# connortannahill/MM-ADMM

Measured on AMD Instinct MI355X. Metric: ADMM iterations/sec on 1M-node 2D mesh; achieved HBM GB/s in SpMV, higher is better.
Workload: dtype f64

## Files before the change

### mm-admm_amd/csrc/host/engine.cpp

```cpp
#include <algorithm>
#include <chrono>
#include <cmath>
#include <cstring>
#include <limits>
#include <memory>
#include <mutex>
#include <string>
#include <vector>

#include "../../../include/mmx_sparse.h"
#include "../kernels/admm_kernels.h"
#include "../kernels/regrid_kernels.h"
#include "comm.h"
#include "common.h"
#include "partition.h"

#define MMX_SP(expr)                                                                     \
  do {                                                                                   \
    const int rc_ = (expr);                                                              \
    if (rc_ != MMADMM_OK) throw ::mmx::Error(rc_, std::string(#expr) + ": " + mmadmm_last_error()); \
  } while (0)

namespace mmx {

// ... 264 lines not shown
  void step(int nIters, double tol, double* Ih, int* itersOut) override {
    if (nIters < 1) throw Error(MMADMM_ERR_INVALID, "step: nIters must be >= 1");
    if (regridEachStep_) regrid(stepsTaken_ * prm_.dt);
    ensureResults(nIters);
    const bool timing = timing_;
    hipEvent_t eStep0 = nullptr, eStep1 = nullptr;
    if (timing) {
      eStep0 = nextEvent();
      MMX_HIP(hipEventRecord(eStep0, st_));
    }
    const double dtOverTau = prm_.dt / prm_.tau;
    const bool fusePred = zFromX_ && fusePred_ && !wave2d_ && !(prm_.grad_use || stepsTaken_ <= 2);
    if (prm_.grad_use || stepsTaken_ <= 2) {
      int nb = 0;
      launch_grad_simplex<D>(m_, x_.p, gs_.p, true, partA_.p, &nb, st_);
      exchange(1);
      launch_predict<D>(m_, 0, gs_.p, x_.p, xPrev_.p, xBar_.p, dtOverTau, st_);
    } else if (!fusePred) {
      launch_predict<D>(m_, 1, nullptr, x_.p, xPrev_.p, xBar_.p, dtOverTau, st_);
    }
    const double* zsrc = stepsTaken_ == 0 ? xPrev_.p : xBar_.p;
    const bool zFromX = zFromX_ && !wave2d_;
    if (!stepTaken_) clearU();
    if (zFromX)
      m_.zx = zsrc;
    else
      launch_gather_z<D>(m_, zsrc, z_.p, st_);
    gcacheValid_ = false;
    if (!zFromX) m_.zx = nullptr;
    StepScalars sc{prm_.tau, prm_.dt * prm_.dt, w_, dtOverTau};
    int nbx = 0, nbp = 0;
    if (fusePred) {
      m_.predPrev = xPrev_.p;
      m_.predBar = xBar_.p;
    }
    PackZX pz;
    if (zFromX) {
      pz.F = F_.p;
      pz.zx = zsrc;
      if (fusePred) {
        pz.x = x_.p;
        pz.xPrev = xPrev_.p;
      }
    }
    xupdateHalo(sc, &nbx, false, false, pz);
    m_.predPrev = m_.predBar = nullptr;
    const bool early = tol >= 0;
    int done = 0;
    double primal = 0, dual = 0;
    const bool deferRed = !early && nIters <= kDeferMax;
    const size_t slice = maxBlocks_ * kNumPartials;
    if (deferRed && partA_.n < slice * nIters) partA_.alloc(slice * std::max(nIters, 10));
    int firstDeferred = 0;
    for (int i = 0; i < nIters; ++i) {
      hipEvent_t a0 = nullptr, a1 = nullptr, b1 = nullptr;
      if (timing) {
        a0 = nextEvent();
        MMX_HIP(hipEventRecord(a0, st_));
      }
      const bool firstProx = !hessComputed_;
      const bool swapB = prox_double_buffered(D, wave2d_) && hessComputed_;
      if (hessComputed_) {
        tiePar_ ^= 1;
        std::swap(m_.tieCount, m_.tieStale);
      }
      launch_prox<D>(m_, !hessComputed_, gcacheValid_, early ? tol / 100 : 1e-3 / 100, x_.p, z_.p, uPtr(), B_.p,
                     swapB ? B2_.p : B_.p, partA_.p + (deferRed ? slice * i : 0), &nbp, st_);
      m_.zx = nullptr;
      if (swapB) std::swap(B_.p, B2_.p);
      gcacheValid_ = true;
      if (timing) {
        a1 = nextEvent();
        MMX_HIP(hipEventRecord(a1, st_));
      }
      hessComputed_ = true;
      stepTaken_ = true;
      const bool resid = early || i == nIters - 1;
      xupdateHalo(sc, &nbx, resid, true, PackZX{});
      if (timing) {
        b1 = nextEvent();
        MMX_HIP(hipEventRecord(b1, st_));
        timed_.push_back({a0, a1, b1});
      }
      if (deferRed) {
        if (firstProx && i < nIters - 1) {
          launch_reduce_partials(partA_.p + slice * i, nbp, res_ + (size_t)i * 2 * kNumPartials, st_, red_);
          firstDeferred = i + 1;
        } else if (i == nIters - 1) {
          const int i0 = firstProx ? i : firstDeferred;
          launch_reduce_steps(partA_.p + slice * i0, slice, nbp, partB_.p, nbx, nIters - i0,
                              res_ + (size_t)i0 * 2 * kNumPartials, st_, red_);
        }
      } else if (resid) {
        launch_reduce_partials2(partA_.p, nbp, res_ + (size_t)i * 2 * kNumPartials, partB_.p, nbx,
                                res_ + (size_t)i * 2 * kNumPartials + kNumPartials, st_, red_);
      } else {
        launch_reduce_partials(partA_.p, nbp, res_ + (size_t)i * 2 * kNumPartials, st_, red_);
      }
      done = i + 1;
      if (early) {
        std::vector<double> rv;
        fetchResults(res_ + (size_t)i * 2 * kNumPartials, 1, rv);
        const double* r = rv.data();
        primal = sqrt(r[kNumPartials + 2]);
        dual = sqrt(r[1]);
        if (r[4] > 0 || (primal < tol && dual < tol)) break;
      }
    }
    MMX_HIP(hipMemcpyAsync(Vp_.p, x_.p, (size_t)nP_ * D * sizeof(double), hipMemcpyDeviceToDevice, st_));
    vpVersion_++;
    if (timing) {
      eStep1 = nextEvent();
      MMX_HIP(hipEventRecord(eStep1, st_));
    }
    fetchResults(res_, done, hostRes_);
    MMX_HIP(hipGetLastError());
    bool bad = false;
    long long bf = 0;
    int mx = 0;
    for (int i = 0; i < done; ++i) {
      const double* r = &hostRes_[(size_t)i * 2 * kNumPartials];
      bad |= r[4] > 0;
      bf += (long long)r[3];
      mx = std::max(mx, (int)r[5]);
    }
    const double* last = &hostRes_[(size_t)(done - 1) * 2 * kNumPartials];
    primal = sqrt(last[kNumPartials + 2]);
    dual = sqrt(last[1]);
    st_stats_.admm_iters += done;
    st_stats_.bfgs_iters += bf;
    st_stats_.max_bfgs = mx;
    st_stats_.last_primal = primal;
    st_stats_.last_dual = dual;
    st_stats_.steps += 1;
    if (timing) {
      stepEv_.push_back({eStep0, eStep1});
      if (evUsed_ >= kEvResolve) resolveTimed();
    }
    stepsTaken_++;
    if (bad) throwBad("in prox");
    if (Ih) *Ih = hostRes_[0];
    if (itersOut) *itersOut = done;
  }

  double eulerStep() override {
    clearInvFlag();
    int nb = 0;
    launch_grad_simplex<D>(m_, x_.p, gs_.p, false, partA_.p, &nb, st_);
    launch_reduce_partials(partA_.p, nb, res_, st_, red_);
    exchange(1);
    launch_euler_apply<D>(m_, gs_.p, x_.p, prm_.dt / prm_.tau, st_);
    std::vector<double> rv;
    fetchResults(res_, 1, rv);
    const double* r = rv.data();
    if (r[4] > 0) throwBad("in the explicit Euler gradient");
    return r[0];
  }

  double backwardEulerStep(double dtBE, double tol, int* newtonOut) override {
    if (nranks_ > 1) throw Error(MMADMM_ERR_INVALID, "backward Euler runs on one rank (no element partition)");
    const auto tStep = Clock::now();
    const int n = nP_ * D;
    ensureJacobian();
    const double dtot = dtBE / prm_.tau;
    const double SAFETY_FAC = 1.0 / 10.0;
    const int MAX_ITERS = 1000;
    clearInvFlag();
    MMX_HIP(hipMemcpyAsync(xn_.p, x_.p, (size_t)n * sizeof(double), hipMemcpyDeviceToDevice, st_));
    int nb = 0, nb2 = 0;
    launch_grad_simplex<D>(m_, x_.p, gs_.p, false, partA_.p, &nb, st_);
    launch_euler_apply<D>(m_, gs_.p, x_.p, dtot, st_);
    if (!beStepTaken_) buildJacobian(dtBE);
    int nIter = 0;
    double Ih = 0.0, normPrev = INFINITY;
    std::vector<double> rv;
    void* mst = nullptr;
    MMX_SP(mmx_matrix_stream(jac_, &mst));
    do {
// ... 808 lines not shown
                      grid_.nz, rgMon_.p, rgTmp_.p, H, st_);
    double* cur = rgTmp_.p;
    double* oth = part ? rgTmp2_.p : gvals_.p;
    for (int it = 0; it < passes; ++it) {
      launch_smooth<D>(cur, oth, grid_.nx, grid_.ny, grid_.nz, widen(R, part ? passes - 1 - it : 0), st_);
      std::swap(cur, oth);
    }
    if (part) {
      launch_box_commit<D>(cur, gvals_.p, D == 3 ? gpad_.p : nullptr, grid_.nx, grid_.ny, grid_.nz, R, st_);
    } else {
      if (cur != gvals_.p)
        MMX_HIP(hipMemcpyAsync(gvals_.p, cur, gvals_.n * sizeof(double), hipMemcpyDeviceToDevice, st_));
      if (D == 3) launch_pad_rows(gvals_.p, (long long)(gvals_.n / 9), gpad_.p, st_);
    }
    st_stats_.regrid_rows = (long long)(H.hi[0] - H.lo[0] + 1) * (H.hi[1] - H.lo[1] + 1) * (H.hi[2] - H.lo[2] + 1);
    st_stats_.regrid_gather_bytes = part ? (double)nranks_ * maxOwned_ * D * sizeof(double) : 0.0;
    st_stats_.regrid_cand = part ? nG : 0;
    MMX_HIP(hipGetLastError());
    gridOnDevice_ = true;
    updateIso();
    m_ = makeView();
    st_stats_.regrids += 1;
  }

  DeviceMesh<D> makeView() const {
    DeviceMesh<D> m{};
    m.nP = nP_;
    m.nF = nF_;
    m.F = F_.p;
    m.sbits = sbits_.p;
    m.nodeInterior = interior_.p;
    m.inc_ptr = incPtr_.p;
    m.inc_off = incOff_.p;
    m.remote = nranks_ > 1 ? remote_.p : nullptr;
    m.tslot = tslotOn_ ? tslot_.p : nullptr;
    m.gcache = gcache_.p;
    m.tieList = tieList_.p;
    m.tieCount = tieCount_.p + tiePar_;
    m.tieStale = tieCount_.p + (tiePar_ ^ 1);
    m.invFlag = tieCount_.p + 2;
    m.nodeOrder = nodeOrder_.p;
    m.xupLo = 0;
    m.xupHi = nP_;
    m.prox2dWave = wave2d_ ? 1 : 0;
    {
      const char* xs = getenv("MMX_XUP_SWEEP");
      m.xupSweep = xs ? std::max(0, atoi(xs)) : (D == 3 ? 1 : 0);
      const char* xc = getenv("MMX_XUP_CH");
      m.xupCh = xc ? atoi(xc) : 8;
    }
    {
      const char* ft = getenv("MMX_FORCE_TIE");
      m.forceTie = ft ? atoi(ft) : 0;
    }
    m.invdiag = invdiag_.p;
    m.Vc = compMesh_ ? Vc_.p : nullptr;
    m.gx = gx_.p;
    m.gy = gy_.p;
    m.gz = (D == 3) ? gz_.p : gy_.p;
    m.gvals = gvals_.p;
    m.gpad = (D == 3) ? gpad_.p : nullptr;
    for (int a = 0; a < 3; ++a) m.gcell[a] = (D == 3) ? gcell_[a].p : nullptr;
    m.giso = iso_ ? giso_.p : nullptr;
    m.gnx = grid_.nx;
    m.gny = grid_.ny;
    m.gnz = grid_.nz;
    m.ghx = grid_.gx[1] - grid_.gx[0];
    m.ghy = grid_.gy[1] - grid_.gy[0];
    m.ghz = (D == 3) ? grid_.gz[1] - grid_.gz[0] : 1.0;
    m.grhx = 1.0 / m.ghx;
    m.grhy = 1.0 / m.ghy;
    m.grhz = 1.0 / m.ghz;
    const int ns[3] = {grid_.nx, grid_.ny, grid_.nz};
    double* A[3] = {&m.gax, &m.gay, &m.gaz};
    double* SP[3] = {&m.gspx, &m.gspy, &m.gspz};
    double* NS[3] = {&m.gnsx, &m.gnsy, &m.gnsz};
    double* RNS[3] = {&m.grnsx, &m.grnsy, &m.grnsz};
    for (int d = 0; d < 3; ++d) {
      const bool on = d < D;
      *A[d] = on ? grid_.lo[d] : 0.0;
      *SP[d] = on ? grid_.hi[d] - grid_.lo[d] : 0.0;
      *NS[d] = on ? (double)ns[d] : 1.0;
      *RNS[d] = 1.0 / *NS[d];
    }
    for (int i = 0; i < D * D; ++i) m.Ehat[i] = EhatH_[i];
    m.powd = powd_;
    m.w = w_;
    m.compMesh = compMesh_ ? 1 : 0;
    return m;
  }

  void ensureResults(int nIters) {
    if (nIters <= resultsCap_) return;
    resultsCap_ = std::max(nIters, 64);
    const size_t n = (size_t)resultsCap_ * 2 * kNumPartials;
    if (nranks_ == 1 && spinWait_) {
      if (resH_) MMX_HIP(hipHostFree(resH_));
      resH_ = nullptr;
      MMX_HIP(hipHostMalloc((void**)&resH_, n * sizeof(double), hipHostMallocMapped));
      MMX_HIP(hipHostGetDevicePointer((void**)&res_, resH_, 0));
    } else {
      results_.alloc(n);
      res_ = results_.p;
    }
  }

// ... 322 lines not shown
```

### mm-admm_amd/csrc/kernels/admm_device.h

```cpp
#pragma once
#include <hip/hip_runtime.h>
#include <stdint.h>

#include "crmath.h"

namespace mmx {

enum : int { BOUNDARY_FREE = 0, BOUNDARY_FIXED = 1, INTERIOR = 2 };

template <int D>
struct GridView {
  const double* gx;
  const double* gy;
  const double* gz;
  const double* vals;
  const double* pad;
  const double* cell[3];
  const double* iso;
  int nx, ny, nz;
  double hx, hy, hz;
  double rhx, rhy, rhz;
  double ax, ay, az, spx, spy, spz, nsx, nsy, nsz, rnsx, rnsy, rnsz;
  unsigned* invFlag;
};
// ... 190 lines not shown
#pragma unroll
    for (int n = 0; n < 9; ++n) f[n] += c[q] * in.r[q][n];
#pragma unroll
  for (int n = 0; n < 9; ++n) mv.m[n / 3][n % 3] = f[n];
}
struct MonIso3 {
  double x0, x1, y0, y1, z0, z1;
  double r[8];
};
__device__ __forceinline__ void monLoad3Iso(const GridView<3>& g, const double* pnt, MonIso3& in) {
  const int xInd = findLimInf(pnt[0], g.ax, g.nx + 1, g.hx, g.rhx);
  const int yInd = findLimInf(pnt[1], g.ay, g.ny + 1, g.hy, g.rhy);
  const int zInd = findLimInf(pnt[2], g.az, g.nz + 1, g.hz, g.rhz);
  const int nx = g.nx;
#ifdef MMX_GRID_RECOMPUTE3
  in.x0 = gridCoord(g.ax, g.spx, g.nsx, g.rnsx, xInd);
  in.x1 = gridCoord(g.ax, g.spx, g.nsx, g.rnsx, xInd + 1);
  in.y0 = gridCoord(g.ay, g.spy, g.nsy, g.rnsy, yInd);
  in.y1 = gridCoord(g.ay, g.spy, g.nsy, g.rnsy, yInd + 1);
  in.z0 = gridCoord(g.az, g.spz, g.nsz, g.rnsz, zInd);
  in.z1 = gridCoord(g.az, g.spz, g.nsz, g.rnsz, zInd + 1);
#else
  in.x0 = g.gx[xInd];
  in.x1 = g.gx[xInd + 1];
  in.y0 = g.gy[yInd];
  in.y1 = g.gy[yInd + 1];
  in.z0 = g.gz[zInd];
  in.z1 = g.gz[zInd + 1];
#endif
  const size_t P = (size_t)(nx + 1) * (g.ny + 1);
  const size_t base = zInd * P + (size_t)yInd * (nx + 1) + xInd;
  const size_t rows[8] = {base, base + 1, base + nx + 1, base + nx + 2,
                          base + P, base + P + 1, base + P + nx + 1, base + P + nx + 2};
#pragma unroll
  for (int q = 0; q < 8; ++q) in.r[q] = g.iso[rows[q]];
}
__device__ __forceinline__ void monEval3Iso(const MonIso3& in, const double* pnt, M<3>& mv) {
  const double xd = (pnt[0] - in.x0) / (in.x1 - in.x0);
  const double yd = (pnt[1] - in.y0) / (in.y1 - in.y0);
  const double zd = (pnt[2] - in.z0) / (in.z1 - in.z0);
  const double c[8] = {(1 - xd) * (1 - yd) * (1 - zd), xd * (1 - yd) * (1 - zd),
                       (1 - xd) * yd * (1 - zd),       xd * yd * (1 - zd),
                       (1 - xd) * (1 - yd) * zd,       xd * (1 - yd) * zd,
                       (1 - xd) * yd * zd,             xd * yd * zd};
  double d = 0.0, o = 0.0;
#pragma unroll
  for (int q = 0; q < 8; ++q) {
    d += c[q] * in.r[q];
    o += c[q] * 0.0;
  }
#pragma unroll
  for (int n = 0; n < 9; ++n) mv.m[n / 3][n % 3] = (n / 3 == n % 3) ? d : o;
}
template <int D>
__device__ __forceinline__ void evalMonitor(const GridView<D>& g, const double* pnt, M<D>& mv) {
  const int xInd = findLimInf(pnt[0], g.ax, g.nx + 1, g.hx, g.rhx);
  const int yInd = findLimInf(pnt[1], g.ay, g.ny + 1, g.hy, g.rhy);
  const int nx = g.nx;
  if constexpr (D == 2) {
#ifdef MMX_GRID_LOAD
    const double xm0 = g.gx[xInd], xm1 = g.gx[xInd + 1], ym0 = g.gy[yInd], ym1 = g.gy[yInd + 1];
#else
    const double xm0 = gridCoord(g.ax, g.spx, g.nsx, g.rnsx, xInd), xm1 = gridCoord(g.ax, g.spx, g.nsx, g.rnsx, xInd + 1);
    const double ym0 = gridCoord(g.ay, g.spy, g.nsy, g.rnsy, yInd), ym1 = gridCoord(g.ay, g.spy, g.nsy, g.rnsy, yInd + 1);
#endif
    const double x = pnt[0], y = pnt[1];
    const double norm = (1 / ((xm1 - xm0) * (ym1 - ym0)));
    const double c0 = norm * (xm1 - x) * (ym1 - y), c1 = norm * (x - xm0) * (ym1 - y);
    const double c2 = norm * (xm1 - x) * (y - ym0), c3 = norm * (x - xm0) * (y - ym0);
    if (g.iso) {
      const double* r0 = g.iso + (size_t)yInd * (nx + 1) + xInd;
      const double* r1 = r0 + (nx + 1);
      const double a = r0[0], b = r0[1], e = r1[0], f = r1[1];
      const double d = c0 * a + c1 * b + c2 * e + c3 * f;
      const double o = c0 * 0.0 + c1 * 0.0 + c2 * 0.0 + c3 * 0.0;
      mv.m[0][0] = d;
      mv.m[0][1] = o;
      mv.m[1][0] = o;
      mv.m[1][1] = d;
      return;
    }
    const double2* r0 = reinterpret_cast<const double2*>(g.vals + ((size_t)yInd * (nx + 1) + xInd) * 4);
    const double2* r1 = reinterpret_cast<const double2*>(g.vals + ((size_t)(yInd + 1) * (nx + 1) + xInd) * 4);
    const double2 a0 = r0[0], a1 = r0[1], b0 = r0[2], b1 = r0[3];
    const double2 e0 = r1[0], e1 = r1[1], f0 = r1[2], f1 = r1[3];
    mv.m[0][0] = c0 * a0.x + c1 * b0.x + c2 * e0.x + c3 * f0.x;
    mv.m[0][1] = c0 * a0.y + c1 * b0.y + c2 * e0.y + c3 * f0.y;
    mv.m[1][0] = c0 * a1.x + c1 * b1.x + c2 * e1.x + c3 * f1.x;
    mv.m[1][1] = c0 * a1.y + c1 * b1.y + c2 * e1.y + c3 * f1.y;
  } else {
    const int zInd = findLimInf(pnt[2], g.az, g.nz + 1, g.hz, g.rhz);
    const double x0 = g.gx[xInd], x1 = g.gx[xInd + 1];
    const double y0 = g.gy[yInd], y1 = g.gy[yInd + 1];
    const double z0 = g.gz[zInd], z1 = g.gz[zInd + 1];
    const double xd = (pnt[0] - x0) / (x1 - x0);
    const double yd = (pnt[1] - y0) / (y1 - y0);
    const double zd = (pnt[2] - z0) / (z1 - z0);
    const double c[8] = {(1 - xd) * (1 - yd) * (1 - zd), xd * (1 - yd) * (1 - zd),
                         (1 - xd) * yd * (1 - zd),       xd * yd * (1 - zd),
                         (1 - xd) * (1 - yd) * zd,       xd * (1 - yd) * zd,
                         (1 - xd) * yd * zd,             xd * yd * zd};
    const size_t P = (size_t)(nx + 1) * (g.ny + 1);
    const size_t base = zInd * P + (size_t)yInd * (nx + 1) + xInd;
    const size_t rows[8] = {base, base + 1, base + nx + 1, base + nx + 2,
                            base + P, base + P + 1, base + P + nx + 1, base + P + nx + 2};
    if (g.iso) {
      double d = 0.0, o = 0.0;
#pragma unroll
      for (int q = 0; q < 8; ++q) {
        d += c[q] * g.iso[rows[q]];
        o += c[q] * 0.0;
      }
#pragma unroll
      for (int n = 0; n < 9; ++n) mv.m[n / 3][n % 3] = (n / 3 == n % 3) ? d : o;
      return;
    }
    double f[9];
#pragma unroll
    for (int n = 0; n < 9; ++n) f[n] = 0.0;
#if MMX_MON_BATCH
    double r[8][10];
#pragma unroll
    for (int q = 0; q < 8; ++q) {
      const double2* rp = reinterpret_cast<const double2*>(g.pad + rows[q] * 10);
#pragma unroll
      for (int e = 0; e < 5; ++e) {
        const double2 v = rp[e];
        r[q][2 * e] = v.x;
        r[q][2 * e + 1] = v.y;
      }
    }
#pragma unroll
    for (int q = 0; q < 8; ++q)
#pragma unroll
      for (int n = 0; n < 9; ++n) f[n] += c[q] * r[q][n];
#else
#pragma unroll
    for (int q = 0; q < 8; ++q) {
      const double2* rp = reinterpret_cast<const double2*>(g.pad + rows[q] * 10);
      double r[10];
#pragma unroll
      for (int e = 0; e < 5; ++e) {
        const double2 v = rp[e];
        r[2 * e] = v.x;
        r[2 * e + 1] = v.y;
      }
#pragma unroll
      for (int n = 0; n < 9; ++n) f[n] += c[q] * r[n];
    }
#endif
#pragma unroll
    for (int n = 0; n < 9; ++n) mv.m[n / 3][n % 3] = f[n];
  }
}

template <int D, bool EXACT>
__device__ __forceinline__ double pow_dp2(double x, bool& tie) {
  if constexpr (D == 2) return cr_pow_p15<EXACT>(x, tie);
  else return cr_pow_p225<EXACT>(x, tie);
}
template <int D, bool EXACT>
__device__ __forceinline__ double pow_dp2m1(double x, bool& tie) {
  if constexpr (D == 2) return cr_pow_p05(x);
  else return cr_pow_p125<EXACT>(x, tie);
}

template <int D, bool GRAD, bool REG, bool EXACT = true>
__device__ __forceinline__ double blockGrad(const GridView<D>& g, const FunctionalConsts<D>& fc,
                                            const double* z, const double* xi, const double* dxpu,
                                            double* grad, double& Igt, double* ghuang = nullptr,
                                            bool* tiep = nullptr) {
  bool tie = false;
  constexpr int K = D * (D + 1);
  const double dFact = (D == 2) ? 2.0 : 6.0;
  M<D> mPre[D + 1], Msum;
  if constexpr (D == 3 && MMX_MON_PIPE) {
    if (g.iso) {
      MonIso3 ja, jb;
      monLoad3Iso(g, &z[0], ja);
      monLoad3Iso(g, &z[3], jb);
      monEval3Iso(ja, &z[0], mPre[0]);
      monLoad3Iso(g, &z[6], ja);
      monEval3Iso(jb, &z[3], mPre[1]);
      monLoad3Iso(g, &z[9], jb);
      monEval3Iso(ja, &z[6], mPre[2]);
      monEval3Iso(jb, &z[9], mPre[3]);
    } else {
      MonIn3 ia, ib;
      monLoad3(g, &z[0], ia);
      monLoad3(g, &z[3], ib);
      monEval3(ia, &z[0], mPre[0]);
      monLoad3(g, &z[6], ia);
      monEval3(ib, &z[3], mPre[1]);
      monLoad3(g, &z[9], ib);
      monEval3(ia, &z[6], mPre[2]);
      monEval3(ib, &z[9], mPre[3]);
    }
  }
#pragma unroll
  for (int i = 0; i < D + 1; i++) {
    if constexpr (!(D == 3 && MMX_MON_PIPE)) evalMonitor<D>(g, &z[i * D], mPre[i]);
#pragma unroll
    for (int r = 0; r < D; ++r)
#pragma unroll
      for (int c = 0; c < D; ++c) Msum.m[r][c] = ((i == 0) ? 0.0 : Msum.m[r][c]) + mPre[i].m[r][c];
  }
  M<D> dmv[D];
#pragma unroll
  for (int j = 0; j < D; ++j)
#pragma unroll
    for (int r = 0; r < D; ++r)
#pragma unroll
      for (int c = 0; c < D; ++c) dmv[j].m[r][c] = mPre[j + 1].m[r][c] - mPre[0].m[r][c];
  M<D> Minv = inverse<D>(Msum);
#pragma unroll
  for (int r = 0; r < D; ++r)
#pragma unroll
    for (int c = 0; c < D; ++c) Minv.m[r][c] = Minv.m[r][c] / ((double)D + 1);
  M<D> E, Ehat;
#pragma unroll
  for (int j = 0; j < D; ++j) {
#pragma unroll
    for (int r = 0; r < D; ++r) {
      E.m[r][j] = z[D * (j + 1) + r] - z[r];
      Ehat.m[r][j] = fc.compMesh ? (xi[D * (j + 1) + r] - xi[r]) : fc.Ehat[r * D + j];
    }
  }
  const double Edet = det<D>(E);
  if (!(Edet > 0)) {
    if (Edet <= 0 && g.invFlag) *g.invFlag = 1u;
    const double nan = __builtin_nan("");
    if constexpr (GRAD) {
#pragma unroll
      for (int i = 0; i < K; ++i) grad[i] = nan;
      if (ghuang)
#pragma unroll
        for (int i = 0; i < K; ++i) ghuang[i] = nan;
    }
    Igt = nan;
    return nan;
  }
  const M<D> Einv = inverse<D>(E);
  const M<D> FJ = mul<D>(Ehat, Einv);
  const double detFJ = det<D>(FJ);
  const double d = (double)D;
  const double p = 1.5;
  const double theta = 1.0 / 3.0;
  const M<D> FJt = transpose<D>(FJ);
  const M<D> MinvJt = mul<D>(Minv, FJt);
  const M<D> JMJt = mul<D>(FJ, MinvJt);
  const double trJMJt = trace<D>(JMJt);
  const double detM = cr_sqrt(1.0 / det<D>(Minv));
  const double tr_dp2 = pow_dp2<D, EXACT>(trJMJt, tie);
  const double G = theta * detM * tr_dp2 + (1.0 - 2.0 * theta) * fc.powd * detM * cr_pow_p15<EXACT>(detFJ / detM, tie);
// ... 105 lines not shown
```

### mm-admm_amd/csrc/kernels/admm_kernels.h

```cpp
#pragma once
#include <hip/hip_runtime.h>
#include <stdint.h>

#include "layout.h"

namespace mmx {

constexpr int kNumPartials = kLayoutPartials;

template <int D>
struct DeviceMesh {
  int nP, nF;
  const int* F;
  const uint8_t* sbits;
  const uint8_t* nodeInterior;
  const int* inc_ptr;
  const int* inc_off;
  const double* remote;
  double* tslot;
  const double* zx;
  double* predPrev;
  double* predBar;
  double* gcache;
  int* tieList;
  unsigned* tieCount;
  unsigned* tieStale;
  unsigned* invFlag;
  int xupCh;
  int xupSweep;
  int forceTie;
  const int* nodeOrder;
  int xupLo, xupHi;
  const double* invdiag;
  const double* Vc;
  const double* gx;
  const double* gy;
  const double* gz;
  const double* gvals;
  const double* gpad;
  const double* gcell[3];
  const double* giso;
  int gnx, gny, gnz;
  double ghx, ghy, ghz, grhx, grhy, grhz;
  double gax, gay, gaz, gspx, gspy, gspz, gnsx, gnsy, gnsz, grnsx, grnsy, grnsz;
  double Ehat[9];
  double powd, w;
  int compMesh;
  int prox2dWave;
};

struct StepScalars {
  double tau, dtsq, w, dt_over_tau;
};

template <int D>
void launch_gather_z(const DeviceMesh<D>& m, const double* x, double* z, hipStream_t st);
template <int D>
void launch_grad_simplex(const DeviceMesh<D>& m, const double* x, double* gs, bool zeroFixed,
                         double* partials, int* nblocks, hipStream_t st);
template <int D>
void launch_predict(const DeviceMesh<D>& m, int mode, const double* gs, double* x, double* xPrev,
                    double* xBar, double dt_over_tau, hipStream_t st);
template <int D>
void launch_xupdate(const DeviceMesh<D>& m, const StepScalars& sc, const double* xBar,
                    const double* z, const double* u, double* x, double* partials, int* nblocks,
                    bool resid, hipStream_t st, bool useTslot = false);
void launch_pad_rows(const double* vals, long long rows, double* pad, hipStream_t st);
template <int D>
void launch_iso_compact(const double* vals, long long points, double* iso, int* notIso, hipStream_t st);
template <int D>
void launch_bkinv_identity(int nF, double* B, hipStream_t st);

bool prox_double_buffered(int D, bool wave2d);
bool prox2d_wave_requested();
template <int D>
void launch_prox(const DeviceMesh<D>& m, bool first, bool useCache, double tol, const double* x, double* z,
                 double* u, const double* Bin, double* Bout, double* partials, int* nblocks, hipStream_t st);
template <int D>
void launch_energy(const DeviceMesh<D>& m, const double* x, double* partials, int* nblocks,
                   hipStream_t st);
template <int D>
void launch_euler_apply(const DeviceMesh<D>& m, const double* gs, double* x, double dt_over_tau,
                        hipStream_t st);
// ... 40 lines not shown
```

### mm-admm_amd/csrc/kernels/admm_kernels.hip

```cpp
#include <hip/hip_runtime.h>

#include <algorithm>
#include <stdexcept>
#include <cstdio>
#include <cstdlib>
#include <string>
#include <vector>

#include "admm_device.h"
#include "admm_kernels.h"

namespace mmx {

constexpr int kBlock = 256;
constexpr int kLdsStride = kBlock + 1;
constexpr int kProxBlock = 64;

__device__ __forceinline__ double wave_sum(double v) {
#pragma unroll
  for (int off = 32; off > 0; off >>= 1) v += __shfl_xor(v, off, 64);
  return v;
}
__device__ __forceinline__ double wave_max(double v) {
#pragma unroll
// ... 555 lines not shown
    double by = row[0] * (ykr[0] * pk[j]);
#pragma unroll
    for (int q = 1; q < K; ++q) by += row[q] * (ykr[q] * pk[j]);
    if constexpr (EXACT) {
      nrow[j] = row[j] + (((c1 * (pki * pk[j])) - by / c2) - (pki * yB[j]) / c2);
    } else {
      eBy = max(eBy, mk_exp(by, 900));
      nrow[j] = row[j] + (((c1 * (pki * pk[j])) - div_mk(by, c2, rc2)) - div_mk(pki * yB[j], c2, rc2));
      fin = cr_fma(nrow[j], 0.0, fin);
    }
  }
#pragma unroll
  for (int j = 0; j < K; ++j) B.set(i, j, nrow[j]);
}

#ifndef MMX_UPD_ROWS
#define MMX_UPD_ROWS 2
#endif
template <int D, bool EXACT, int UR, class BA, int K>
__device__ __forceinline__ void bfgs_update_rows(BA& B, int i, const double (&pki)[UR], const double (&row)[UR][K],
                                                 const double (&yk)[K], const double (&pk)[K], const double (&yB)[K],
                                                 double c1, double c2, double rc2, unsigned& eBy, double& fin) {
  double nrow[UR][K], ykr[K];
#pragma unroll
  for (int q = 0; q < K; ++q) {
    ykr[q] = yk[q];
    asm volatile("" : "+v"(ykr[q]));
  }
#pragma unroll
  for (int j = 0; j < K; ++j) {
    double yp[K];
#pragma unroll
    for (int q = 0; q < K; ++q) yp[q] = ykr[q] * pk[j];
#pragma unroll
    for (int u = 0; u < UR; ++u) {
      double by = row[u][0] * yp[0];
#pragma unroll
      for (int q = 1; q < K; ++q) by += row[u][q] * yp[q];
      if constexpr (EXACT) {
        nrow[u][j] = row[u][j] + (((c1 * (pki[u] * pk[j])) - by / c2) - (pki[u] * yB[j]) / c2);
      } else {
        eBy = max(eBy, mk_exp(by, 900));
        nrow[u][j] = row[u][j] + (((c1 * (pki[u] * pk[j])) - div_mk(by, c2, rc2)) - div_mk(pki[u] * yB[j], c2, rc2));
        fin = cr_fma(nrow[u][j], 0.0, fin);
      }
    }
  }
#pragma unroll
  for (int u = 0; u < UR; ++u)
#pragma unroll
    for (int j = 0; j < K; ++j) B.set(i + u, j, nrow[u][j]);
}

template <int D, class BA, bool EXACT = true>
__device__ __forceinline__ int bfgs_iterations(BA B, const GridView<D>& g, const FunctionalConsts<D>& fc,
                                               double* z, const double* xi, const double* dx, double* G,
                                               unsigned fixedBits, double tol, bool& bad, double* gcache,
                                               bool* tie = nullptr) {
  constexpr int K = D * (D + 1);
  constexpr int kPipe = BA::kPipe;
  int iter;
  for (iter = 0; iter < 50; iter++) {
    B.fresh();
    double pk[K];
    double rn[kPipe > 0 ? kPipe : 1][K];
    constexpr bool kCarry = BA::kCarry && kPipe > 0;
    double rc[kPipe > 0 ? kPipe : 1][K];
    const bool pre = BA::kPre && iter == 0;
    constexpr int kP1 = BA::kPipe1;
    double rn1[kP1 > 0 ? kP1 : 1][K];
    start_rows<K, kP1>(B, rn1, pre ? BA::kHeld : 0);
#pragma unroll
    for (int i = 0; i < K; ++i) {
      MMX_ROW_FENCE(BA);
      double row[K];
      next_row<K, kP1>(B, i, row, rn1, pre);
      if constexpr (BA::kHeld > 0) {
        if (!pre && i < BA::kHeld)
#pragma unroll
          for (int j = 0; j < K; ++j) B.holdRow(i, j, row[j]);
      }
      if constexpr (kCarry) {
        if (i >= BA::kHeld && i < BA::kHeld + kPipe)
#pragma unroll
          for (int j = 0; j < K; ++j) rc[i - BA::kHeld][j] = row[j];
      }
      double sacc = (-row[0]) * G[0];
#pragma unroll
      for (int j = 1; j < K; ++j) sacc += (-row[j]) * G[j];
      pk[i] = sacc;
    }
    MMX_ROW_FENCE(BA);
    if constexpr (BA::kPipe > 0 && !EXACT) {
      if (iter == 0) WPROF(2, pk[K - 1]);
    }
#pragma unroll
    for (int i = 0; i < K; ++i) z[i] += pk[i];
    double G1[K], Igt;
    {
      const double e = blockGrad<D, true, true, EXACT>(g, fc, z, xi, dx, G1, Igt, gcache, tie);
      bad |= (e != e);
    }
    if constexpr (BA::kPipe > 0 && !EXACT) {
      if (iter == 0) WPROF(3, G1[K - 1]);
    }
    if constexpr (!EXACT) {
      if (*tie) break;
    }
    zeroFixed<D>(G1, fixedBits);
    double Ix = 0;
#pragma unroll
    for (int i = 0; i < K; i++) Ix += __builtin_fabs(G1[i]);
    double yk[K];
#pragma unroll
    for (int i = 0; i < K; ++i) yk[i] = G1[i] - G[i];
    double c2 = pk[0] * yk[0];
#pragma unroll
    for (int i = 1; i < K; ++i) c2 += pk[i] * yk[i];
    B.fresh();
    double yBy = 0.0, yB[K];
    constexpr int kP2 = BA::kPipe2 > kPipe ? BA::kPipe2 : kPipe;
    double rn2[kP2 > 0 ? kP2 : 1][K];
    if constexpr (kCarry) {
#pragma unroll
      for (int d = 0; d < kPipe; ++d)
#pragma unroll
        for (int j = 0; j < K; ++j) rn2[d][j] = rc[d][j];
#pragma unroll
      for (int d = kPipe; d < kP2; ++d)
        if (BA::kHeld + d < K) load_row<K>(B, BA::kHeld + d, rn2[d]);
    } else {
      start_rows<K, kP2>(B, rn2, BA::kHeld);
    }
#pragma unroll
    for (int i = 0; i < K; ++i) {
      MMX_ROW_FENCE(BA);
      double row[K];
      next_row<K, kP2>(B, i, row, rn2, true);
      if constexpr (kCarry) {
        if (i >= BA::kHeld && i < BA::kHeld + kPipe)
#pragma unroll
          for (int j = 0; j < K; ++j) rc[i - BA::kHeld][j] = row[j];
      }
      double by = row[0] * yk[0];
#pragma unroll
      for (int j = 1; j < K; ++j) by += row[j] * yk[j];
      yBy = (i == 0) ? yk[0] * by : yBy + yk[i] * by;
#pragma unroll
      for (int j = 0; j < K; ++j) yB[j] = (i == 0) ? yk[0] * row[j] : yB[j] + yk[i] * row[j];
    }
    MMX_ROW_FENCE(BA);
    const double c1 = (c2 + yBy) / cr_pow_2(c2);
    if constexpr (BA::kPipe > 0 && !EXACT) {
// ... 158 lines not shown
  for (int i = 0; i < K; ++i) {
    zs[zu_i<D>(i)] = z[i];
    un[i] = dx[i] - z[i];
    us[zu_i<D>(i)] = un[i];
    const double d = z[i] - zold[i];
    dual2 += d * d;
  }
  write_tslot<D>(m, s, z, un);
#pragma unroll
  for (int i = 0; i < K * K; ++i) Bout[bidx<D>(s, i)] = B[i];
  pv[0] = Ihsave;
  pv[1] = dual2;
  pv[3] = (double)its;
  pv[4] = bad ? 1.0 : 0.0;
  pv[5] = (double)its;
}

template <int D, bool FIRST, int ISO = -1>
__global__ void __launch_bounds__(kBlock) k_prox(DeviceMesh<D> m, double tol, const double* __restrict__ x,
                                                  double* __restrict__ zg, double* __restrict__ ug,
                                                  const double* Bin, double* Bout, double* __restrict__ partials,
                                                  int useCache) {
  const int s = blockIdx.x * kBlock + threadIdx.x;
  double pv[6] = {0, 0, 0, 0, 0, 0};
  if (s < m.nF) prox_simplex<D, FIRST, ISO>(m, tol, x, zg, ug, Bin, Bout, useCache != 0, s, pv);
  block_partials<6>(pv, partials);
}

__device__ __forceinline__ void rearm_tie_queue(unsigned* tieStale) {
  if (blockIdx.x == 0 && threadIdx.x == 0) *tieStale = 0u;
}
template <int D, int BS>
__global__ void __launch_bounds__(BS) k_prox_fix(DeviceMesh<D> m, double tol, const double* __restrict__ x,
                                                 double* __restrict__ zg, double* __restrict__ ug,
                                                 const double* Bin, double* Bout, double* __restrict__ partials) {
  const unsigned n = *m.tieCount;
  for (unsigned i = blockIdx.x; i < n; i += gridDim.x) {
    const int b = m.tieList[i];
    const int s = b * BS + (int)threadIdx.x;
    double pv[6] = {0, 0, 0, 0, 0, 0};
    if (s < m.nF) prox_simplex<D, false>(m, tol, x, zg, ug, Bin, Bout, false, s, pv);
    block_partials<6, BS>(pv, partials, b);
    __syncthreads();
  }
  rearm_tie_queue(m.tieStale);
}

typedef double v2nt __attribute__((ext_vector_type(2)));
#ifndef MMX_ZU_NT
#define MMX_ZU_NT 0
#endif
#ifndef MMX_LDS_DMA
#define MMX_LDS_DMA 0
#endif
template <int D, int BS>
__global__ void __launch_bounds__(BS, 2) k_prox_lds(DeviceMesh<D> m, double tol, const double* __restrict__ x,
                                                        double* __restrict__ zg, double* __restrict__ ug,
                                                        double* __restrict__ Bg, double* __restrict__ partials,
                                                        int useCache) {
  constexpr int K = D * (D + 1), KK = K * K;
  static_assert(BS % 64 == 0, "whole wave blocks per chunk");
  __shared__ __attribute__((aligned(16))) double lds[KK * BS];
  const int tid = threadIdx.x;
  const int lb = (int)blockIdx.x;
  const int s0 = lb * BS;
  const int nIn = min(BS, m.nF - s0);
  const bool act = tid < nIn;
  const int s = act ? s0 + tid : s0;
  int f[D + 1];
  loadVerts<D>(m, s, f);
  const unsigned fixedBits = m.sbits[s] & 0xF;
  double* zs = zg + zu_base<D>(s);
  double* us = ug + zu_base<D>(s);
  double* gc = m.gcache + (size_t)s * K;
  double z[K], z0[K], dx[K], gcv[K];
  if (m.zx)
    gatherX<D>(m.zx, f, z);
  else
#pragma unroll
    for (int i = 0; i < K; ++i) z[i] = zs[zu_i<D>(i)];
#pragma unroll
  for (int i = 0; i < K; ++i) {
    z0[i] = z[i];
    dx[i] = us[zu_i<D>(i)];
  }
  if (useCache) {
#pragma unroll
    for (int i = 0; i < K; ++i) gcv[i] = gc[i];
  }
  double* chunk = Bg + (size_t)s0 * KK;
  constexpr int NL = KK / 2;
  v2nt cv[MMX_LDS_DMA ? 1 : NL];
  if constexpr (!MMX_LDS_DMA) {
#pragma unroll
    for (int r = 0; r < NL; ++r) cv[r] = __builtin_nontemporal_load(reinterpret_cast<const v2nt*>(chunk) + tid + r * BS);
  }
  double xi[K], dxv[K];
  loadXi<D>(m, f, xi);
  gatherX<D>(x, f, dxv);
  if constexpr (MMX_LDS_DMA) {
    __builtin_amdgcn_sched_barrier(0);
    const char* src = reinterpret_cast<const char*>(chunk) + tid * 16;
    const int wofs = __builtin_amdgcn_readfirstlane((tid >> 6) * 1024);
#pragma unroll
    for (int r = 0; r < NL; ++r)
      __builtin_amdgcn_global_load_lds(src + r * BS * 16,
                                       (__attribute__((address_space(3))) void*)(reinterpret_cast<char*>(lds) + wofs + r * BS * 16),
                                       16, 0, 0);
    __builtin_amdgcn_sched_barrier(0);
    __builtin_amdgcn_s_waitcnt(0);
  } else {
#pragma unroll
    for (int r = 0; r < NL; ++r) reinterpret_cast<v2nt*>(lds)[tid + r * BS] = cv[r];
  }
#pragma unroll
  for (int i = 0; i < K; ++i) dx[i] = dxv[i] + dx[i];
  __syncthreads();
  double pv[6] = {0, 0, 0, 0, 0, 0};
  bool tie = false;
  if (act) {
    const GridView<D> g = gridOf<D>(m);
    const FunctionalConsts<D> fc = constsOf<D>(m);
    double G[K], Igt;
    bool bad = false;
    entry_grad<D, false>(g, fc, z, xi, dx, gcv, useCache != 0, G, Igt, bad, &tie);
    zeroFixed<D>(G, fixedBits);
    const double Ihsave = Igt;
    LdsB<K, 64> Bacc{lds + (tid >> 6) * KK * 64 + (tid & 63)};
    const int its =
        tie ? 0 : bfgs_iterations<D, LdsB<K, 64>, false>(Bacc, g, fc, z, xi, dx, G, fixedBits, tol, bad, gc, &tie);
    double dual2 = 0.0;
#pragma unroll
    for (int i = 0; i < K; ++i) {
      const double d = z[i] - z0[i];
      dual2 += d * d;
    }
    pv[0] = Ihsave;
    pv[1] = dual2;
    pv[3] = (double)its;
    pv[4] = bad ? 1.0 : 0.0;
    pv[5] = (double)its;
  }
  if (m.forceTie > 0 && tid == 0 && (int)((unsigned)lb % (unsigned)m.forceTie) == 0) tie = true;
  if (__syncthreads_or(tie ? 1 : 0)) {
    if (tid == 0) m.tieList[atomicAdd(m.tieCount, 1u)] = lb;
    return;
  }
  if (act) {
    double un[K];
#pragma unroll
    for (int i = 0; i < K; ++i) {
      un[i] = dx[i] - z[i];
      if constexpr (MMX_ZU_NT) {
        __builtin_nontemporal_store(z[i], &zs[zu_i<D>(i)]);
        __builtin_nontemporal_store(un[i], &us[zu_i<D>(i)]);
      } else {
        zs[zu_i<D>(i)] = z[i];
        us[zu_i<D>(i)] = un[i];
      }
    }
    write_tslot<D>(m, s, z, un);
  }
#pragma unroll
  for (int r = 0; r < NL; ++r)
    __builtin_nontemporal_store(reinterpret_cast<const v2nt*>(lds)[tid + r * BS], reinterpret_cast<v2nt*>(chunk) + tid + r * BS);
  block_partials<6, BS>(pv, partials, lb);
}

#ifndef MMX_WAVE_OCC
#define MMX_WAVE_OCC 1
#endif
#ifndef MMX_WAVE_OCC2
#define MMX_WAVE_OCC2 2
#endif
#ifndef MMX_WAVE_PERSIST
#define MMX_WAVE_PERSIST 0
#endif
#ifndef MMX_HELD_DMA_CPOL
#define MMX_HELD_DMA_CPOL 2
#endif
#ifndef MMX_WAVE_XCD
#define MMX_WAVE_XCD 1
#endif
// ... 1540 lines not shown
```

Measured before the change: 2572.

## Prefetch monitor-grid cell values early in 2D prox kernel as a hint

At the start of the 2D LDS prox kernel, each thread speculatively loads the iso monitor values for the cell containing each vertex of z. These loads are issued alongside the B-chunk and x gathers, so their latency overlaps. In the first BFGS iteration, the monitor evaluation reuses the prefetched values when the cell index matches and otherwise falls back to a global load. This adds twelve registers per thread and extra speculative loads, which may hurt occupancy or waste bandwidth on misses. The change also reuses the previous iteration's end event as the next start event in timing mode, and adds an optional hit-count probe.

```diff
diff --git a/mm-admm_amd/csrc/host/engine.cpp b/mm-admm_amd/csrc/host/engine.cpp
--- a/mm-admm_amd/csrc/host/engine.cpp
+++ b/mm-admm_amd/csrc/host/engine.cpp
@@ -340,11 +340,15 @@
     const size_t slice = maxBlocks_ * kNumPartials;
     if (deferRed && partA_.n < slice * nIters) partA_.alloc(slice * std::max(nIters, 10));
     int firstDeferred = 0;
+    hipEvent_t prevEnd = nullptr;
     for (int i = 0; i < nIters; ++i) {
       hipEvent_t a0 = nullptr, a1 = nullptr, b1 = nullptr;
       if (timing) {
-        a0 = nextEvent();
-        MMX_HIP(hipEventRecord(a0, st_));
+        a0 = prevEnd;
+        if (!a0) {
+          a0 = nextEvent();
+          MMX_HIP(hipEventRecord(a0, st_));
+        }
       }
       const bool firstProx = !hessComputed_;
       const bool swapB = prox_double_buffered(D, wave2d_) && hessComputed_;
@@ -370,8 +374,10 @@
         MMX_HIP(hipEventRecord(b1, st_));
         timed_.push_back({a0, a1, b1});
       }
+      prevEnd = b1;
       if (deferRed) {
         if (firstProx && i < nIters - 1) {
+          prevEnd = nullptr;
           launch_reduce_partials(partA_.p + slice * i, nbp, res_ + (size_t)i * 2 * kNumPartials, st_, red_);
           firstDeferred = i + 1;
         } else if (i == nIters - 1) {
@@ -380,9 +386,11 @@
                               res_ + (size_t)i0 * 2 * kNumPartials, st_, red_);
         }
       } else if (resid) {
+        prevEnd = nullptr;
         launch_reduce_partials2(partA_.p, nbp, res_ + (size_t)i * 2 * kNumPartials, partB_.p, nbx,
                                 res_ + (size_t)i * 2 * kNumPartials + kNumPartials, st_, red_);
       } else {
+        prevEnd = nullptr;
         launch_reduce_partials(partA_.p, nbp, res_ + (size_t)i * 2 * kNumPartials, st_, red_);
       }
       done = i + 1;
@@ -412,6 +420,14 @@
       bf += (long long)r[3];
       mx = std::max(mx, (int)r[5]);
     }
+#ifdef MMX_HINT_PROBE
+    {
+      double hits = 0;
+      for (int i = 0; i < done; ++i) hits += hostRes_[(size_t)i * 2 * kNumPartials + 2];
+      fprintf(stderr, "[hint-probe] step %lld: %.0f hits of %.0f lookups in %d proxes\n", (long long)stepsTaken_, hits,
+              3.0 * nF_ * done, done);
+    }
+#endif
     const double* last = &hostRes_[(size_t)(done - 1) * 2 * kNumPartials];
     primal = sqrt(last[kNumPartials + 2]);
     dual = sqrt(last[1]);
@@ -1326,6 +1342,9 @@
     {
       const char* ft = getenv("MMX_FORCE_TIE");
       m.forceTie = ft ? atoi(ft) : 0;
+      const char* mh = getenv("MMX_MON_HINT");
+      m.monHint = mh ? atoi(mh) : 1;
+      if (m.monHint < 0 || m.monHint > 3) m.monHint = 1;
     }
     m.invdiag = invdiag_.p;
     m.Vc = compMesh_ ? Vc_.p : nullptr;
diff --git a/mm-admm_amd/csrc/kernels/admm_device.h b/mm-admm_amd/csrc/kernels/admm_device.h
--- a/mm-admm_amd/csrc/kernels/admm_device.h
+++ b/mm-admm_amd/csrc/kernels/admm_device.h
@@ -266,8 +266,36 @@
 #pragma unroll
   for (int n = 0; n < 9; ++n) mv.m[n / 3][n % 3] = (n / 3 == n % 3) ? d : o;
 }
-template <int D>
-__device__ __forceinline__ void evalMonitor(const GridView<D>& g, const double* pnt, M<D>& mv) {
+struct MonHint2 {
+  int cell[3];
+  double v[12];
+#ifdef MMX_HINT_PROBE
+  mutable int hits;
+#endif
+};
+__device__ __forceinline__ void monHintVertex(const GridView<2>& g, const double* z, int mode, int* cell, double* v) {
+  int xInd = findLimInf(z[0], g.ax, g.nx + 1, g.hx, g.rhx);
+  int yInd = findLimInf(z[1], g.ay, g.ny + 1, g.hy, g.rhy);
+  if (mode == 2) xInd = min(xInd + 1, g.nx - 1);
+  if (mode == 3) yInd = min(yInd + 1, g.ny - 1);
+  const int c = yInd * (g.nx + 1) + xInd;
+  const double* r0 = g.iso + c;
+  const double* r1 = r0 + (g.nx + 1);
+  *cell = c;
+  v[0] = r0[0];
+  v[1] = r0[1];
+  v[2] = r1[0];
+  v[3] = r1[1];
+}
+__device__ __forceinline__ void monHintRequest(const GridView<2>& g, const double* z, int mode, MonHint2& h) {
+  monHintVertex(g, &z[0], mode, &h.cell[0], &h.v[0]);
+  monHintVertex(g, &z[2], mode, &h.cell[1], &h.v[4]);
+  monHintVertex(g, &z[4], mode, &h.cell[2], &h.v[8]);
+}
+
+template <int D, bool HINT = false>
+__device__ __forceinline__ void evalMonitor(const GridView<D>& g, const double* pnt, M<D>& mv,
+                                            const MonHint2* hint = nullptr, int hv = 0, bool useHint = false) {
   const int xInd = findLimInf(pnt[0], g.ax, g.nx + 1, g.hx, g.rhx);
   const int yInd = findLimInf(pnt[1], g.ay, g.ny + 1, g.hy, g.rhy);
   const int nx = g.nx;
@@ -285,7 +313,21 @@
     if (g.iso) {
       const double* r0 = g.iso + (size_t)yInd * (nx + 1) + xInd;
       const double* r1 = r0 + (nx + 1);
-      const double a = r0[0], b = r0[1], e = r1[0], f = r1[1];
+      double a, b, e, f;
+      if constexpr (HINT) {
+        if (useHint && hint->cell[hv] == yInd * (nx + 1) + xInd) {
+          a = hint->v[4 * hv], b = hint->v[4 * hv + 1], e = hint->v[4 * hv + 2], f = hint->v[4 * hv + 3];
+#ifdef MMX_HINT_PROBE
+          hint->hits++;
+#endif
+        } else {
+          typedef const __attribute__((address_space(1))) double* gptr;
+          const gptr q0 = (gptr)r0, q1 = (gptr)r1;
+          a = q0[0], b = q0[1], e = q1[0], f = q1[1];
+        }
+      } else {
+        a = r0[0], b = r0[1], e = r1[0], f = r1[1];
+      }
       const double d = c0 * a + c1 * b + c2 * e + c3 * f;
       const double o = c0 * 0.0 + c1 * 0.0 + c2 * 0.0 + c3 * 0.0;
       mv.m[0][0] = d;
@@ -379,11 +421,13 @@
   else return cr_pow_p125<EXACT>(x, tie);
 }
 
-template <int D, bool GRAD, bool REG, bool EXACT = true>
+template <int D, bool GRAD, bool REG, bool EXACT = true, bool HINT = false>
 __device__ __forceinline__ double blockGrad(const GridView<D>& g, const FunctionalConsts<D>& fc,
                                             const double* z, const double* xi, const double* dxpu,
                                             double* grad, double& Igt, double* ghuang = nullptr,
-                                            bool* tiep = nullptr) {
+                                            bool* tiep = nullptr, const MonHint2* hint = nullptr,
+                                            bool useHint = false) {
+  static_assert(!HINT || D == 2, "the monitor-cell hint is 2D only");
   bool tie = false;
   constexpr int K = D * (D + 1);
   const double dFact = (D == 2) ? 2.0 : 6.0;
@@ -411,9 +455,14 @@
       monEval3(ib, &z[9], mPre[3]);
     }
   }
+  if constexpr (HINT) {
+    evalMonitor<D, true>(g, &z[0], mPre[0], hint, 0, useHint);
+    evalMonitor<D, true>(g, &z[D], mPre[1], hint, 1, useHint);
+    evalMonitor<D, true>(g, &z[2 * D], mPre[2], hint, 2, useHint);
+  }
 #pragma unroll
   for (int i = 0; i < D + 1; i++) {
-    if constexpr (!(D == 3 && MMX_MON_PIPE)) evalMonitor<D>(g, &z[i * D], mPre[i]);
+    if constexpr (!(D == 3 && MMX_MON_PIPE) && !HINT) evalMonitor<D>(g, &z[i * D], mPre[i]);
 #pragma unroll
     for (int r = 0; r < D; ++r)
 #pragma unroll
diff --git a/mm-admm_amd/csrc/kernels/admm_kernels.h b/mm-admm_amd/csrc/kernels/admm_kernels.h
--- a/mm-admm_amd/csrc/kernels/admm_kernels.h
+++ b/mm-admm_amd/csrc/kernels/admm_kernels.h
@@ -29,6 +29,7 @@
   int xupCh;
   int xupSweep;
   int forceTie;
+  int monHint;
   const int* nodeOrder;
   int xupLo, xupHi;
   const double* invdiag;
diff --git a/mm-admm_amd/csrc/kernels/admm_kernels.hip b/mm-admm_amd/csrc/kernels/admm_kernels.hip
--- a/mm-admm_amd/csrc/kernels/admm_kernels.hip
+++ b/mm-admm_amd/csrc/kernels/admm_kernels.hip
@@ -631,11 +631,11 @@
     for (int j = 0; j < K; ++j) B.set(i + u, j, nrow[u][j]);
 }
 
-template <int D, class BA, bool EXACT = true>
+template <int D, class BA, bool EXACT = true, bool HINT = false>
 __device__ __forceinline__ int bfgs_iterations(BA B, const GridView<D>& g, const FunctionalConsts<D>& fc,
                                                double* z, const double* xi, const double* dx, double* G,
                                                unsigned fixedBits, double tol, bool& bad, double* gcache,
-                                               bool* tie = nullptr) {
+                                               bool* tie = nullptr, const MonHint2* hint = nullptr) {
   constexpr int K = D * (D + 1);
   constexpr int kPipe = BA::kPipe;
   int iter;
@@ -677,7 +677,7 @@
     for (int i = 0; i < K; ++i) z[i] += pk[i];
     double G1[K], Igt;
     {
-      const double e = blockGrad<D, true, true, EXACT>(g, fc, z, xi, dx, G1, Igt, gcache, tie);
+      const double e = blockGrad<D, true, true, EXACT, HINT>(g, fc, z, xi, dx, G1, Igt, gcache, tie, hint, iter == 0);
       bad |= (e != e);
     }
     if constexpr (BA::kPipe > 0 && !EXACT) {
@@ -942,6 +942,9 @@
 #endif
 #ifndef MMX_LDS_DMA
 #define MMX_LDS_DMA 0
+#endif
+#ifndef MMX_MON_HINT_BUILD
+#define MMX_MON_HINT_BUILD 1
 #endif
 template <int D, int BS>
 __global__ void __launch_bounds__(BS, 2) k_prox_lds(DeviceMesh<D> m, double tol, const double* __restrict__ x,
@@ -985,6 +988,19 @@
 #pragma unroll
     for (int r = 0; r < NL; ++r) cv[r] = __builtin_nontemporal_load(reinterpret_cast<const v2nt*>(chunk) + tid + r * BS);
   }
+  constexpr bool kHint = (D == 2) && MMX_MON_HINT_BUILD == 1;
+  constexpr bool kTouch = (D == 2) && MMX_MON_HINT_BUILD == 2;
+  MonHint2 hint;
+#ifdef MMX_HINT_PROBE
+  hint.hits = 0;
+#endif
+  if constexpr (kHint || kTouch) {
+    if (m.giso && m.monHint > 0) {
+      monHintRequest(gridOf<D>(m), z, m.monHint, hint);
+    } else {
+      hint.cell[0] = hint.cell[1] = hint.cell[2] = -1;
+    }
+  }
   double xi[K], dxv[K];
   loadXi<D>(m, f, xi);
   gatherX<D>(x, f, dxv);
@@ -1006,6 +1022,11 @@
 #pragma unroll
   for (int i = 0; i < K; ++i) dx[i] = dxv[i] + dx[i];
   __syncthreads();
+  if constexpr (kTouch) {
+    if (hint.cell[0] >= 0)
+#pragma unroll
+      for (int i = 0; i < 12; ++i) asm volatile("" ::"v"(hint.v[i]));
+  }
   double pv[6] = {0, 0, 0, 0, 0, 0};
   bool tie = false;
   if (act) {
@@ -1018,7 +1039,12 @@
     const double Ihsave = Igt;
     LdsB<K, 64> Bacc{lds + (tid >> 6) * KK * 64 + (tid & 63)};
     const int its =
-        tie ? 0 : bfgs_iterations<D, LdsB<K, 64>, false>(Bacc, g, fc, z, xi, dx, G, fixedBits, tol, bad, gc, &tie);
+        tie ? 0
+            : bfgs_iterations<D, LdsB<K, 64>, false, kHint>(Bacc, g, fc, z, xi, dx, G, fixedBits, tol, bad, gc, &tie,
+                                                            kHint ? &hint : nullptr);
+#ifdef MMX_HINT_PROBE
+    if constexpr (kHint) pv[2] = (double)hint.hits;
+#endif
     double dual2 = 0.0;
 #pragma unroll
     for (int i = 0; i < K; ++i) {
```

After: 2640 (median of 6 runs). 2.6% higher.
